# ChenYutongTHU/humannerf

Hardware: AMD Instinct MI355X
Metric: rendered rays/sec (128 samples/ray) at 512x512 (higher is better)
Workload: dtype f32-equivalent: split-f16 hi+lo operands, 3 f16 MFMAs, fp32 accumulate; 1 GPU; BASELINE configs[1]: 512x512 freeview frame, 262144 rays x 128 samples, eval, perturb=0, all 11 outputs of the reference Network.forward; seeded random weights of the default architecture; samples_per_ray=128, ray_chunk=32768, mlp_mode=f16x3, parallelism=frames sharded over 1 GPU(s), no collective

## Files before the change

### humannerf_amd/csrc/hnrf_mlp_f16.hip

```cpp
#include "hnrf_common.h"
#include "hnrf_sincos.h"
#include "hnrf_lds_dma.h"

namespace hnrf {

typedef float f32x16 __attribute__((ext_vector_type(16)));
typedef float f32x2 __attribute__((ext_vector_type(2)));
typedef _Float16 h16x8 __attribute__((ext_vector_type(8)));
typedef _Float16 h16x2 __attribute__((ext_vector_type(2)));

constexpr int RING = 3;
constexpr float LO_SCALE = 2048.0f;
constexpr float LO_INV = 1.0f / 2048.0f;

enum { PE16_NONE = 0, PE16_CANONICAL = 1, PE16_NONRIGID = 2 };

enum { SV_NONE = 0,
       SV_ACT = 1,
       SV_DZ = 2,
       SV_PE = 3,
       SV_ACT_H = 4,
       SV_DZ_H = 5 };
__host__ __device__ constexpr bool sv_fwd(int s) { return s == SV_ACT || s == SV_ACT_H; }
__host__ __device__ constexpr bool sv_bwd(int s) { return s == SV_DZ || s == SV_DZ_H; }
// ... 92 lines not shown
    }
    *reinterpret_cast<h16x2*>(dst) = h16x2{outv[0], outv[1]};
}

constexpr int64_t KB = 1024;
constexpr int CNL16_NB_L0 = 8, CNL16_NB_MID = 32, CNL16_NB_L5 = 40;
constexpr int64_t CNL16_L0 = 0;
constexpr int64_t CNL16_L1 = CNL16_L0 + 8 * CNL16_NB_L0 * KB;
constexpr int64_t CNL16_L5 = CNL16_L1 + 4 * 8 * CNL16_NB_MID * KB;
constexpr int64_t CNL16_L6 = CNL16_L5 + 8 * CNL16_NB_L5 * KB;
constexpr int64_t CNL16_OUT = CNL16_L6 + 2 * 8 * CNL16_NB_MID * KB;
constexpr int64_t CNL16_BIAS = CNL16_OUT + CNL16_NB_MID * KB;
constexpr int CNL16_BIAS_LDS = 8 * 1024;
constexpr int64_t CNL16_BYTES = CNL16_BIAS + 9 * 1024;
constexpr int CNL16_SLAB = 40 * 1024;
constexpr int NR16_NB_L0 = 8, NR16_NB_MID = 16, NR16_NB_L4 = 24;
constexpr int64_t NR16_L0 = 0;
constexpr int64_t NR16_L1 = NR16_L0 + 4 * NR16_NB_L0 * KB;
constexpr int64_t NR16_L4 = NR16_L1 + 3 * 4 * NR16_NB_MID * KB;
constexpr int64_t NR16_L5 = NR16_L4 + 4 * NR16_NB_L4 * KB;
constexpr int64_t NR16_OUT = NR16_L5 + 4 * NR16_NB_MID * KB;
constexpr int64_t NR16_BIAS = NR16_OUT + NR16_NB_MID * KB;
constexpr int NR16_BIAS_LDS = 3 * 1024;
constexpr int64_t NR16_BYTES = NR16_BIAS + 4 * 1024;
constexpr int NR16_SLAB = 32 * 1024;
constexpr int64_t CNL16_STATUS = CNL16_BIAS + 8 * 1024 + 512;
constexpr int64_t NR16_STATUS = NR16_BIAS + 3 * 1024 + 512;
constexpr int PE_STASH = 32 * 1024;

typedef __attribute__((address_space(3))) char lds_char;
typedef __attribute__((address_space(3))) h16x8 lds_h16x8;
typedef float f32x4 __attribute__((ext_vector_type(4)));
typedef __attribute__((address_space(3))) f32x4 lds_f32x4;

__device__ __forceinline__ h16x8 lds_ld8(unsigned addr) { return *reinterpret_cast<const lds_h16x8*>((size_t)addr); }
__device__ __forceinline__ f32x4 lds_ld4f(unsigned addr) { return *reinterpret_cast<const lds_f32x4*>((size_t)addr); }
__device__ __forceinline__ void lds_st8(unsigned addr, h16x8 v) { *reinterpret_cast<lds_h16x8*>((size_t)addr) = v; }

__device__ __forceinline__ void slab_issue(const char* gsrc, unsigned lds_addr, int nblocks, int wave, int nw = 4) {
    const unsigned voff = lane_now() * 16;
    for (int b = wave; b < nblocks; b += nw) dma_piece(gsrc + b * 1024, voff, lds_addr + b * 1024);
}

__device__ __forceinline__ void tile_sync(int keep) {
    wait_dma_keep(keep);
    __builtin_amdgcn_s_barrier();
    asm volatile("" ::: "memory");
}

template <bool ULO>
__device__ __forceinline__ void split8(const float (&v)[8], h16x8& hi, h16x8& lo) {
#pragma unroll
    for (int i = 0; i < 4; ++i) {
        const f32x2 p = {v[2 * i], v[2 * i + 1]};
        const h16x2 hh = __builtin_convertvector(p, h16x2);
        const f32x2 rem = ULO ? f32x2{p[0] - (float)hh[0], p[1] - (float)hh[1]}
                              : f32x2{fmaf((float)hh[0], -LO_SCALE, p[0] * LO_SCALE), fmaf((float)hh[1], -LO_SCALE, p[1] * LO_SCALE)};
// ... 152 lines not shown
        epi_core<ACT_MASK_SEL, ULO>(pacc1, pacc2, I, sc->mask[(T) >> 1] >> (16 * ((T) & 1)), 0, oh[2 * (T) + ((I) >> 2)],      \
                                    ol[2 * (T) + ((I) >> 2)], x0, x1);                                                         \
        save_pair_b(*sc, T, I, x0, x1);                                                                                        \
    } else if constexpr (SAVE == SV_DZ_H) {                                                                                    \
        float x0, x1;                                                                                                          \
        const h16x2 hh = epi_core<ACT_MASK_AND, ULO>(pacc1, pacc2, I, sc->mask[(T) >> 1], 8 * ((T) & 1) + (I),                 \
                                                     oh[2 * (T) + ((I) >> 2)], ol[2 * (T) + ((I) >> 2)], x0, x1);              \
        store_pair_h(rowh, cxh, svu, T, I, hh);                                                                                \
    } else if constexpr (SAVE == SV_PE) {                                                                                      \
        sc->fout[16 * (T) + 2 * (I)] = fmaf(pacc2[2 * (I)], LO_INV, pacc1[2 * (I)]);                                           \
        sc->fout[16 * (T) + 2 * (I) + 1] = fmaf(pacc2[2 * (I) + 1], LO_INV, pacc1[2 * (I) + 1]);                               \
    } else                                                                                                                     \
        epi_pair<RELU>(pacc1, I, oh[2 * (T) + ((I) >> 2)], ol[2 * (T) + ((I) >> 2)], p.sat, p.guard);

template <int NT, int TPS, int NKA, int NKB, bool RELU, int SAVE = 0, bool PEND_IN = false, bool DEFER = false,
          int NW = 4, int NB, int NO>
__device__ __forceinline__ void layer16(Pipe& p, int nb1, int nb2, h16x8 (&bh)[NB], h16x8 (&bl)[NB],
                                        h16x8 (&oh)[NO], h16x8 (&ol)[NO], float (&last)[16], SaveCtx* sc = nullptr,
                                        f32x16* pend = nullptr) {
    static_assert(!(PEND_IN || DEFER) || SAVE == SV_NONE, "deferred epilogues exist in the inference form only");
    static_assert(!PEND_IN || NKB >= 2, "a pending tile fills the last two hidden fragments");
    static_assert(NB >= (NKB > 0 ? NKB : 1) && NO >= 2 * NT && NT % TPS == 0, "bad layer shape");
    constexpr int NK = NKA + NKB;
    constexpr int NBLK = 2 * NK;
    constexpr int NS = NT / TPS;
    constexpr int PFK = NK < 4 ? NK : 4;
    static_assert((NBLK * TPS) % NW == 0, "every wave must issue the same number of DMA pieces per slab");
    constexpr bool ULO = !sv_lifted(SAVE);
    constexpr int ACT = RELU ? ACT_RELU : ACT_NONE;
    static_assert(ULO || NT > 1, "the head layers exist in the forward kernels only");
    f32x16 pacc1 = {0.f, 0.f, 0.f, 0.f, 0.f, 0.f, 0.f, 0.f, 0.f, 0.f, 0.f, 0.f, 0.f, 0.f, 0.f, 0.f};
    f32x16 pacc2 = pacc1;
    f32x16 nbias = pacc1;
    uint32_t bw[(NT + 1) / 2];
    _Float16* const rowh = (SAVE == SV_ACT_H || SAVE == SV_DZ_H) ? sc->rowh : nullptr;
    const int cxh = (SAVE == SV_ACT_H || SAVE == SV_DZ_H) ? sc->cx : 0;
    unsigned svu = 0u;
#pragma unroll
    for (int i = 0; i < (NT + 1) / 2; ++i) bw[i] = 0u;
#pragma unroll
    for (int s = 0; s < NS; ++s) {
        const int nissue = (s + 2 < NS) ? NBLK * TPS : (s + 2 == NS ? nb1 : nb2);
        const unsigned slot2 = p.ph == 0 ? 2 : p.ph - 1;
        const int dcnt = nissue / NW;
        const char* dsrc = p.gi + p.wave * dcnt * 1024;
        const unsigned ddst = p.lds_base + p.ring_off + slot2 * p.slab_bytes + p.wave * dcnt * 1024;
        p.gi += nissue * 1024;
#pragma unroll
        for (int tt = 0; tt < TPS; ++tt) {
            const int t = s * TPS + tt;
            const unsigned lane = lane_now();
            unsigned cur = p.lds_base + p.ring_off + p.ph * p.slab_bytes + tt * (NBLK * 1024) + lane * 16;
            unsigned pe = p.lds_base + p.pe_off + p.wave * (PE_STASH / 4) + lane * 16;
            asm volatile("" : "+v"(cur), "+v"(pe));
            f32x16 acc1 = {0.f, 0.f, 0.f, 0.f, 0.f, 0.f, 0.f, 0.f, 0.f, 0.f, 0.f, 0.f, 0.f, 0.f, 0.f, 0.f};
            f32x16 acc2 = acc1;
            if (NT > 1 && sv_has_bias(SAVE)) {
                if (t == 0) {
                    const unsigned bp = p.lds_base + p.bias_off + tt * 128 + (lane >> 5) * 16;
// ... 41 lines not shown
                if (ULO) acc1 = __builtin_amdgcn_mfma_f32_32x32x16_f16(wh, xl, acc1, 0, 0, 0);
                else acc2 = __builtin_amdgcn_mfma_f32_32x32x16_f16(wh, xl, acc2, 0, 0, 0);
                if (ULO) acc1 = __builtin_amdgcn_mfma_f32_32x32x16_f16(wl, xh, acc1, 0, 0, 0);
                else acc2 = __builtin_amdgcn_mfma_f32_32x32x16_f16(wl, xh, acc2, 0, 0, 0);
                if (NT > 1 && sv_has_bias(SAVE) && ks == NK - 1 && t + 1 < NT) {
                    const unsigned bn = p.lds_base + p.bias_off + (tt + 1) * 128 + (lane >> 5) * 16;
                    const f32x4 b0 = lds_ld4f(bn), b1 = lds_ld4f(bn + 32), b2 = lds_ld4f(bn + 64), b3 = lds_ld4f(bn + 96);
                    nbias = f32x16{b0.x, b0.y, b0.z, b0.w, b1.x, b1.y, b1.z, b1.w,
                                   b2.x, b2.y, b2.z, b2.w, b3.x, b3.y, b3.z, b3.w};
                }
                {
                    constexpr int MAXP = (TPS * NK - 1) < 10 ? (TPS * NK - 1) : 10;
                    const int i = tt * NK + ks;
                    if (i >= 0 && i < MAXP) {
                        if (s + 2 < NS) {
                            if (i < NBLK * TPS / NW) dma_run_piece(dsrc, lane * 16, ddst, i);
                        } else if (i < dcnt) {
                            dma_run_piece(dsrc, lane * 16, ddst, i);
                        }
                    }
                }
                if (PEND_IN && t == 0) {
#pragma unroll
                    for (int i = 0; i < 8; ++i)
                        if ((i * (NK - 1)) / 8 == ks) {
                            epi_pair<true>(*pend, i, bh[NKB - 2 + (i >> 2)], bl[NKB - 2 + (i >> 2)], p.sat, p.guard);
                            asm volatile("" : "+v"(bh[NKB - 2 + (i >> 2)]), "+v"(bl[NKB - 2 + (i >> 2)]));
                        }
                }
                if (t > 0) {
#pragma unroll
// ... 8 lines not shown
                __builtin_amdgcn_sched_group_barrier(0x002, 6, 0);
                __builtin_amdgcn_sched_group_barrier(0x008, 1, 0);
                __builtin_amdgcn_sched_group_barrier(0x100, 2, 0);
                __builtin_amdgcn_sched_group_barrier(0x002, 5, 0);
                __builtin_amdgcn_sched_group_barrier(0x008, 1, 0);
                __builtin_amdgcn_sched_group_barrier(0x002, 8, 0);
                __builtin_amdgcn_sched_barrier(0);
            }
#ifdef HNRF_STAMP
            { const unsigned long long t1 = __builtin_readcyclecounter(); p.sum_k += t1 - p.t_last; p.t_last = t1; }
#endif
            pacc1 = acc1;
            pacc2 = acc2;
        }
        const int n_st = (sv_fwd(SAVE) || sv_bwd(SAVE)) ? 4 * (s == 0 ? TPS - 1 : TPS) : 0;
        tile_sync(nissue / NW + n_st);
        p.ph = p.ph == RING - 1 ? 0 : p.ph + 1;
        p.bias_off += TPS * 128;
    }
    if (NT == 1) {
#pragma unroll
        for (int r = 0; r < 16; ++r) last[r] = pacc1[r];
    } else if (DEFER) {
        *pend = pacc1;
    } else {
#pragma unroll
        for (int i = 0; i < 8; ++i) {
            HNRF_TILE_EPILOGUE_PAIR(NT - 1, i)
        }
        if constexpr (sv_fwd(SAVE)) {
#pragma unroll
            for (int i = 0; i < (NT + 1) / 2; ++i) sc->bits[i] = bw[i];
        }
    }
}

#undef HNRF_TILE_EPILOGUE_PAIR

template <int NT, int TPS, int NKA, int NKB, bool RELU, int NB, int NO>
__device__ __forceinline__ void layer16x2(Pipe& p, unsigned stash_per_wave, int nb1, int nb2,
                                          const h16x8 (&bh)[2][NB], const h16x8 (&bl)[2][NB], h16x8 (&oh)[2][NO],
                                          h16x8 (&ol)[2][NO], float (&last)[2][16]) {
    static_assert(NB >= (NKB > 0 ? NKB : 1) && NO >= 2 * NT && NT % TPS == 0, "bad layer shape");
    constexpr int NK = NKA + NKB;
    constexpr int NBLK = 2 * NK;
    constexpr int NS = NT / TPS;
    constexpr int PFK = NK < 4 ? NK : 4;
    static_assert((NBLK * TPS) % 4 == 0, "every wave must issue the same number of DMA pieces per slab");
    const f32x16 zero = {0.f, 0.f, 0.f, 0.f, 0.f, 0.f, 0.f, 0.f, 0.f, 0.f, 0.f, 0.f, 0.f, 0.f, 0.f, 0.f};
    f32x16 pacc[2] = {zero, zero};
#pragma unroll
    for (int s = 0; s < NS; ++s) {
        const int nissue = (s + 2 < NS) ? NBLK * TPS : (s + 2 == NS ? nb1 : nb2);
        const unsigned slot2 = p.ph == 0 ? 2 : p.ph - 1;
        const int dcnt = nissue / 4;
        const char* dsrc = p.gi + p.wave * dcnt * 1024;
        const unsigned ddst = p.lds_base + p.ring_off + slot2 * p.slab_bytes + p.wave * dcnt * 1024;
        p.gi += nissue * 1024;
#pragma unroll
        for (int tt = 0; tt < TPS; ++tt) {
            const int t = s * TPS + tt;
            const unsigned lane = lane_now();
            unsigned cur = p.lds_base + p.ring_off + p.ph * p.slab_bytes + tt * (NBLK * 1024) + lane * 16;
            unsigned pe = p.lds_base + p.pe_off + p.wave * stash_per_wave + lane * 16;
            asm volatile("" : "+v"(cur), "+v"(pe));
            f32x16 acc[2] = {zero, zero};
            if (NT > 1) {
                const unsigned bp = p.lds_base + p.bias_off + tt * 128 + (lane >> 5) * 16;
                const f32x4 b0 = lds_ld4f(bp), b1 = lds_ld4f(bp + 32), b2 = lds_ld4f(bp + 64), b3 = lds_ld4f(bp + 96);
                acc[0] = f32x16{b0.x, b0.y, b0.z, b0.w, b1.x, b1.y, b1.z, b1.w,
                                 b2.x, b2.y, b2.z, b2.w, b3.x, b3.y, b3.z, b3.w};
                acc[1] = acc[0];
            }
            h16x8 qwh[PFK], qwl[PFK], qxh[2][PFK], qxl[2][PFK];
#pragma unroll
            for (int i = 0; i < PFK; ++i) {
                qwh[i] = lds_ld8(cur + (2 * i) * 1024);
                qwl[i] = lds_ld8(cur + (2 * i + 1) * 1024);
                if (i < NKA) {
#pragma unroll
                    for (int g = 0; g < 2; ++g) {
                        qxh[g][i] = lds_ld8(pe + g * (stash_per_wave / 2) + (2 * i) * 1024);
                        qxl[g][i] = lds_ld8(pe + g * (stash_per_wave / 2) + (2 * i + 1) * 1024);
                    }
                }
            }
            __builtin_amdgcn_sched_barrier(0);
#pragma unroll
            for (int ks = 0; ks < NK; ++ks) {
                const int q = ks % PFK;
                const h16x8 wh = qwh[q], wl = qwl[q];
                h16x8 xh[2], xl[2];
#pragma unroll
                for (int g = 0; g < 2; ++g) {
                    if (ks < NKA) {
                        xh[g] = qxh[g][q];
                        xl[g] = qxl[g][q];
                    } else {
                        const int ib = ks - NKA < NB ? ks - NKA : 0;
                        xh[g] = bh[g][ib];
                        xl[g] = bl[g][ib];
                    }
                }
                if (ks + PFK < NK) {
                    qwl[q] = lds_ld8(cur + (2 * (ks + PFK) + 1) * 1024);
                    if (ks + PFK < NKA) {
#pragma unroll
                        for (int g = 1; g >= 0; --g) qxl[g][q] = lds_ld8(pe + g * (stash_per_wave / 2) + (2 * (ks + PFK) + 1) * 1024);
                    }
                    qwh[q] = lds_ld8(cur + (2 * (ks + PFK)) * 1024);
                    if (ks + PFK < NKA) {
#pragma unroll
                        for (int g = 1; g >= 0; --g) qxh[g][q] = lds_ld8(pe + g * (stash_per_wave / 2) + (2 * (ks + PFK)) * 1024);
                    }
                }
#pragma unroll
                for (int g = 0; g < 2; ++g) {
                    acc[g] = __builtin_amdgcn_mfma_f32_32x32x16_f16(wh, xh[g], acc[g], 0, 0, 0);
                    acc[g] = __builtin_amdgcn_mfma_f32_32x32x16_f16(wh, xl[g], acc[g], 0, 0, 0);
                    acc[g] = __builtin_amdgcn_mfma_f32_32x32x16_f16(wl, xh[g], acc[g], 0, 0, 0);
                }
                {
                    constexpr int MAXP = (TPS * NK - 1) < 10 ? (TPS * NK - 1) : 10;
                    const int i = tt * NK + ks;
                    if (i >= 0 && i < MAXP) {
                        if (s + 2 < NS) {
                            if (i < NBLK * TPS / 4) dma_run_piece(dsrc, lane * 16, ddst, i);
                        } else if (i < dcnt) {
                            dma_run_piece(dsrc, lane * 16, ddst, i);
                        }
                    }
                }
                if (t > 0) {
#pragma unroll
                    for (int j = 0; j < 16; ++j)
                        if ((j * NK) / 16 == ks) {
                            const int g = j >> 3, i = j & 7;
                            epi_pair<RELU>(pacc[g], i, oh[g][2 * (t - 1) + (i >> 2)], ol[g][2 * (t - 1) + (i >> 2)], p.sat, p.guard);
                            asm volatile("" : "+v"(oh[g][2 * (t - 1) + (i >> 2)]), "+v"(ol[g][2 * (t - 1) + (i >> 2)]));
                        }
                }
                __builtin_amdgcn_sched_group_barrier(0x008, 1, 0);
                __builtin_amdgcn_sched_group_barrier(0x002, 6, 0);
                __builtin_amdgcn_sched_group_barrier(0x008, 1, 0);
                __builtin_amdgcn_sched_group_barrier(0x100, 2, 0);
                __builtin_amdgcn_sched_group_barrier(0x002, 5, 0);
                __builtin_amdgcn_sched_group_barrier(0x008, 1, 0);
                __builtin_amdgcn_sched_group_barrier(0x100, 2, 0);
                __builtin_amdgcn_sched_group_barrier(0x002, 5, 0);
                __builtin_amdgcn_sched_group_barrier(0x008, 1, 0);
                __builtin_amdgcn_sched_group_barrier(0x002, 6, 0);
                __builtin_amdgcn_sched_group_barrier(0x008, 1, 0);
                __builtin_amdgcn_sched_group_barrier(0x100, 2, 0);
                __builtin_amdgcn_sched_group_barrier(0x002, 5, 0);
                __builtin_amdgcn_sched_group_barrier(0x008, 1, 0);
                __builtin_amdgcn_sched_group_barrier(0x002, 8, 0);
                __builtin_amdgcn_sched_barrier(0);
            }
#pragma unroll
            for (int g = 0; g < 2; ++g) pacc[g] = acc[g];
        }
        tile_sync(nissue / 4);
        p.ph = p.ph == RING - 1 ? 0 : p.ph + 1;
        p.bias_off += TPS * 128;
    }
#pragma unroll
    for (int g = 0; g < 2; ++g) {
        if (NT == 1) {
#pragma unroll
            for (int r = 0; r < 16; ++r) last[g][r] = pacc[g][r];
        } else {
#pragma unroll
            for (int i = 0; i < 8; ++i)
                epi_pair<RELU>(pacc[g], i, oh[g][2 * (NT - 1) + (i >> 2)], ol[g][2 * (NT - 1) + (i >> 2)], p.sat, p.guard);
        }
    }
}

__device__ __forceinline__ Pipe pipe_start(const char* packed, int64_t bias_img_off, int bias_bytes, int slab_bytes,
                                           int nb0, int nb1, char* smem, int stash_bytes = PE_STASH, int nw = 4) {
    Pipe p;
    p.wave = __builtin_amdgcn_readfirstlane(threadIdx.x >> 6);
    p.lds_base = __builtin_amdgcn_readfirstlane((unsigned)(size_t)(lds_char*)smem);
    p.pe_off = bias_bytes;
    p.ring_off = bias_bytes + stash_bytes;
    p.slab_bytes = slab_bytes;
    p.ph = 0;
    p.bias_off = 0;
    p.sat = 0ull;
    p.guard = false;
#ifdef HNRF_STAMP
    p.t_last = __builtin_readcyclecounter();
// ... 95 lines not shown
    if (h == 0 && slot < P)
        raw[sample] = make_float4(fmaf(last[0], hs, ob[0]), fmaf(last[1], hs, ob[1]), fmaf(last[2], hs, ob[2]), fmaf(last[3], hs, ob[3]));
    if constexpr (SAVE == SV_NONE && GUARD) raise_f16_range(packed, CNL16_STATUS, p.sat);
#ifdef HNRF_STAMP
    if (threadIdx.x == 0 && blockIdx.x < 4096) {
        const unsigned long long te = __builtin_readcyclecounter();
        unsigned long long* dbg = (unsigned long long*)(const_cast<char*>(packed) + CNL16_BYTES);
        dbg[blockIdx.x * 4 + 0] = p.sum_k; dbg[blockIdx.x * 4 + 1] = p.sum_b + (te - p.t_last);
    }
#endif
}

constexpr int NR16W8_SLAB = 24 * 1024;
constexpr int NR16W8_STASH = 64 * 1024;

template <int SAVE, int NW = 4>
__global__ __launch_bounds__(64 * NW) void nonrigid_f16x3_kernel(const float* __restrict__ x_skel,
                                                             const float* __restrict__ hann_w,
                                                             const char* __restrict__ packed, int64_t P,
                                                             float* __restrict__ xyz, float* __restrict__ offsets,
                                                             const int* __restrict__ idx,
                                                             const int* __restrict__ count,
                                                             float* __restrict__ pe_out, float* __restrict__ acts,
                                                             uint32_t* __restrict__ relu_bits) {
    extern __shared__ __attribute__((aligned(16))) char smem[];
    if (idx != nullptr) {
        P = *count;
        if ((int64_t)blockIdx.x * (32 * NW) >= P) return;
    }
    static_assert(NW == 4 || NW == 8, "waves per workgroup");
    constexpr bool W8 = NW == 8;
    Pipe p = W8 ? pipe_start(packed, NR16_BIAS, NR16_BIAS_LDS, NR16W8_SLAB, 2 * NR16_NB_L0, 2 * NR16_NB_L0, smem, NR16W8_STASH, 8)
                : pipe_start(packed, NR16_BIAS, NR16_BIAS_LDS, NR16_SLAB, 4 * NR16_NB_L0, 2 * NR16_NB_MID, smem);
    const int lane = threadIdx.x & 63, h = lane >> 5;
    const int64_t slot = ((int64_t)blockIdx.x * NW + p.wave) * 32 + (lane & 31);
    const int64_t sclamp = slot < P ? slot : P - 1;
    const int64_t sidx = idx ? (int64_t)idx[sclamp] : sclamp;
    const int64_t sample = slot < P ? sidx : P;

    const float x[3] = {x_skel[sidx * 3 + 0], x_skel[sidx * 3 + 1], x_skel[sidx * 3 + 2]};
    float pev[32];
    pe_sincos_shared<6>(x, h, pev);
#pragma unroll
    for (int a = 0; a < 18; ++a) pev[a] *= hann_w[a / 3];
#pragma unroll
    for (int a = 18; a < 32; ++a) pev[a] = 0.f;
#pragma unroll
    for (int ks = 0; ks < 4; ++ks) {
        const float v[8] = {pev[8 * ks], pev[8 * ks + 1], pev[8 * ks + 2], pev[8 * ks + 3],
                            pev[8 * ks + 4], pev[8 * ks + 5], pev[8 * ks + 6], pev[8 * ks + 7]};
        stash_pe<true>(p, ks, v);
    }
    SaveCtx sc;
    if constexpr (SAVE) {
        sc.row = acts + sidx * 128 + 4 * h;
        sc.rowh = reinterpret_cast<_Float16*>(acts) + (slot >> 5) * (128 * 32) + h * 128;
        sc.cx = (lane & 31) ^ (4 * h);
        sc.bits = relu_bits + sidx * 4 + 2 * h;
        if constexpr (SAVE == SV_ACT_H) {
            _Float16* ph = reinterpret_cast<_Float16*>(pe_out) + sidx * 64;
#pragma unroll
            for (int a = 0; a < 18; ++a) ph[pe_col16(PE16_NONRIGID, a, h)] = (_Float16)pev[a];
#pragma unroll
            for (int a = 18; a < 32; ++a) ph[36 + 2 * (a - 18) + h] = (_Float16)0.f;
        } else {
#pragma unroll
            for (int a = 0; a < 18; ++a) pe_out[sidx * 36 + pe_col16(PE16_NONRIGID, a, h)] = pev[a];
        }
    }
    const int64_t act_stride = P * 128, bit_stride = P * 4;
    const int64_t acth_stride = (int64_t)gridDim.x * (32 * NW) * 128;
    tile_sync(0);

    h16x8 hA_h[8], hA_l[8], hB_h[8], hB_l[8];
    float last[16];
    h16x8 dh[2], dl[2];
    if constexpr (W8) {
        constexpr int MID = NR16_NB_MID, L4B = NR16_NB_L4;
#define HNRF_NEXT_LAYER if constexpr (SAVE) { sc.row += act_stride; sc.rowh += acth_stride; sc.bits += bit_stride; }
        layer16<4, 2, 4, 0, true, SAVE, false, false, 8>(p, MID, MID, hB_h, hB_l, hA_h, hA_l, last, &sc);
        HNRF_NEXT_LAYER
        layer16<4, 1, 0, 8, true, SAVE, false, false, 8>(p, MID, MID, hA_h, hA_l, hB_h, hB_l, last, &sc);
        HNRF_NEXT_LAYER
        layer16<4, 1, 0, 8, true, SAVE, false, false, 8>(p, MID, MID, hB_h, hB_l, hA_h, hA_l, last, &sc);
        HNRF_NEXT_LAYER
        layer16<4, 1, 0, 8, true, SAVE, false, false, 8>(p, L4B, L4B, hA_h, hA_l, hB_h, hB_l, last, &sc);
        HNRF_NEXT_LAYER
        layer16<4, 1, 4, 8, true, SAVE, false, false, 8>(p, MID, MID, hB_h, hB_l, hA_h, hA_l, last, &sc);
        HNRF_NEXT_LAYER
        layer16<4, 1, 0, 8, true, SAVE, false, false, 8>(p, MID, 0, hA_h, hA_l, hB_h, hB_l, last, &sc);
#undef HNRF_NEXT_LAYER
        layer16<1, 1, 0, 8, false, 0, false, false, 8>(p, 0, 0, hB_h, hB_l, dh, dl, last);
    } else {
    layer16<4, 4, 4, 0, true, SAVE>(p, 0 , 2 * NR16_NB_MID, hB_h, hB_l, hA_h, hA_l, last, &sc);
    if constexpr (SAVE) { sc.row += act_stride; sc.rowh += acth_stride; sc.bits += bit_stride; }
    layer16<4, 2, 0, 8, true, SAVE>(p, 2 * NR16_NB_MID, 2 * NR16_NB_MID, hA_h, hA_l, hB_h, hB_l, last, &sc);
    if constexpr (SAVE) { sc.row += act_stride; sc.rowh += acth_stride; sc.bits += bit_stride; }
    layer16<4, 2, 0, 8, true, SAVE>(p, 2 * NR16_NB_MID, 2 * NR16_NB_MID, hB_h, hB_l, hA_h, hA_l, last, &sc);
    if constexpr (SAVE) { sc.row += act_stride; sc.rowh += acth_stride; sc.bits += bit_stride; }
    layer16<4, 2, 0, 8, true, SAVE>(p, NR16_NB_L4, NR16_NB_L4, hA_h, hA_l, hB_h, hB_l, last, &sc);
    if constexpr (SAVE) { sc.row += act_stride; sc.rowh += acth_stride; sc.bits += bit_stride; }
    layer16<4, 1, 4, 8, true, SAVE>(p, 2 * NR16_NB_MID, 2 * NR16_NB_MID, hB_h, hB_l, hA_h, hA_l, last, &sc);
    if constexpr (SAVE) { sc.row += act_stride; sc.rowh += acth_stride; sc.bits += bit_stride; }
    layer16<4, 2, 0, 8, true, SAVE>(p, NR16_NB_MID, 0, hA_h, hA_l, hB_h, hB_l, last, &sc);
    layer16<1, 1, 0, 8, false, 0>(p, 0, 0, hB_h, hB_l, dh, dl, last);
    }
    const float* ob = reinterpret_cast<const float*>(packed + NR16_BIAS + NR16_BIAS_LDS);
    const float hs = ob[8];
    if (h == 0 && slot < P) {
        const float o0 = fmaf(last[0], hs, ob[0]), o1 = fmaf(last[1], hs, ob[1]), o2 = fmaf(last[2], hs, ob[2]);
        xyz[sample * 3 + 0] = x[0] + o0;
        xyz[sample * 3 + 1] = x[1] + o1;
        xyz[sample * 3 + 2] = x[2] + o2;
        if (offsets) {
            offsets[sample * 3 + 0] = o0;
            offsets[sample * 3 + 1] = o1;
            offsets[sample * 3 + 2] = o2;
        }
    }
}

constexpr int NR16X2_SLAB = 24 * 1024;
constexpr int NR16X2_STASH = 64 * 1024;

template <bool GUARD>
__global__ __launch_bounds__(256) void nonrigid_f16x3_x2_kernel(const float* __restrict__ x_skel,
                                                                const float* __restrict__ hann_w,
                                                                const char* __restrict__ packed, int64_t P,
                                                                float* __restrict__ xyz, float* __restrict__ offsets,
                                                                const int* __restrict__ idx,
                                                                const int* __restrict__ count) {
    extern __shared__ __attribute__((aligned(16))) char smem[];
    if (idx != nullptr) {
        P = *count;
        if ((int64_t)blockIdx.x * 256 >= P) return;
    }
    Pipe p = pipe_start(packed, NR16_BIAS, NR16_BIAS_LDS, NR16X2_SLAB, 2 * NR16_NB_L0, 2 * NR16_NB_L0, smem,
                        NR16X2_STASH);
    p.guard = GUARD;
    constexpr unsigned SPW = NR16X2_STASH / 4;
    const int lane = threadIdx.x & 63, h = lane >> 5;
    int64_t sidx[2];
    bool live[2];
    float x[2][3];
#pragma unroll
    for (int g = 0; g < 2; ++g) {
        const int64_t slot = ((int64_t)blockIdx.x * 4 + p.wave) * 64 + g * 32 + (lane & 31);
        const int64_t sclamp = slot < P ? slot : P - 1;
        sidx[g] = idx ? (int64_t)idx[sclamp] : sclamp;
        live[g] = slot < P;
#pragma unroll
        for (int a = 0; a < 3; ++a) x[g][a] = x_skel[sidx[g] * 3 + a];
    }
#pragma unroll
    for (int g = 0; g < 2; ++g) {
        float pev[32];
        pe_sincos_shared<6>(x[g], h, pev);
#pragma unroll
        for (int a = 0; a < 18; ++a) pev[a] *= hann_w[a / 3];
#pragma unroll
        for (int a = 18; a < 32; ++a) pev[a] = 0.f;
        const unsigned pe = p.lds_base + p.pe_off + p.wave * SPW + g * (SPW / 2) + lane_now() * 16;
#pragma unroll
        for (int ks = 0; ks < 4; ++ks) {
            const float v[8] = {pev[8 * ks], pev[8 * ks + 1], pev[8 * ks + 2], pev[8 * ks + 3],
                                pev[8 * ks + 4], pev[8 * ks + 5], pev[8 * ks + 6], pev[8 * ks + 7]};
            h16x8 hi, lo;
            split8<true>(v, hi, lo);
            lds_st8(pe + (2 * ks) * 1024, hi);
            lds_st8(pe + (2 * ks + 1) * 1024, lo);
        }
    }
    tile_sync(0);

    h16x8 hA_h[2][8], hA_l[2][8], hB_h[2][8], hB_l[2][8];
    float last[2][16];
    constexpr int MID = NR16_NB_MID, L4B = NR16_NB_L4;
    layer16x2<4, 2, 4, 0, true>(p, SPW, MID, MID, hB_h, hB_l, hA_h, hA_l, last);
    layer16x2<4, 1, 0, 8, true>(p, SPW, MID, MID, hA_h, hA_l, hB_h, hB_l, last);
    layer16x2<4, 1, 0, 8, true>(p, SPW, MID, MID, hB_h, hB_l, hA_h, hA_l, last);
    layer16x2<4, 1, 0, 8, true>(p, SPW, L4B, L4B, hA_h, hA_l, hB_h, hB_l, last);
    layer16x2<4, 1, 4, 8, true>(p, SPW, MID, MID, hB_h, hB_l, hA_h, hA_l, last);
    layer16x2<4, 1, 0, 8, true>(p, SPW, MID, 0, hA_h, hA_l, hB_h, hB_l, last);
    h16x8 dh[2][2], dl[2][2];
    layer16x2<1, 1, 0, 8, false>(p, SPW, 0, 0, hB_h, hB_l, dh, dl, last);
    const float* ob = reinterpret_cast<const float*>(packed + NR16_BIAS + NR16_BIAS_LDS);
    const float hs = ob[8];
#pragma unroll
    for (int g = 0; g < 2; ++g) {
        if (h == 0 && live[g]) {
            const float o0 = fmaf(last[g][0], hs, ob[0]), o1 = fmaf(last[g][1], hs, ob[1]), o2 = fmaf(last[g][2], hs, ob[2]);
            xyz[sidx[g] * 3 + 0] = x[g][0] + o0;
            xyz[sidx[g] * 3 + 1] = x[g][1] + o1;
            xyz[sidx[g] * 3 + 2] = x[g][2] + o2;
            if (offsets) {
                offsets[sidx[g] * 3 + 0] = o0;
                offsets[sidx[g] * 3 + 1] = o1;
                offsets[sidx[g] * 3 + 2] = o2;
            }
        }
    }
    if constexpr (GUARD) raise_f16_range(packed, NR16_STATUS, p.sat);
}

struct PackBwd16 {
    const float* W;
    int n_out, n_in;
    int NT, NK;
    int row_kind;
    int col0;
    int head;
    int64_t off;
    const float* amax;
};
// ... 340 lines not shown
    d[5] = PackLayer16{w[5], b[5], 256, 319, 8, 4, 16, PE16_CANONICAL, 0, 63, 0, CNL16_L5, CNL16_BIAS + 5 * 1024, 0};
    for (int l = 6; l <= 7; ++l)
        d[l] = PackLayer16{w[l], b[l], 256, 256, 8, 0, 16, PE16_NONE, 0, 0, 0,
                           CNL16_L6 + (l - 6) * 8 * CNL16_NB_MID * KB, CNL16_BIAS + l * 1024, 0};
    d[8] = PackLayer16{w[8], b[8], 4, 256, 1, 0, 16, PE16_NONE, 0, 0, 0, CNL16_OUT, CNL16_BIAS + 8 * 1024, 1};
    return launch_pack16(d, 9, nullptr, out, st);
}

int nonrigid16_pack(const float* const* w, const float* const* b, const float* cond, void* packed, hipStream_t st) {
    char* out = (char*)packed;
    if (hipMemsetAsync(out + NR16_BIAS, 0, 4 * 1024, st) != hipSuccess) {
        set_error("hnrf_nonrigid_pack: memset failed");
        return HNRF_E_LAUNCH;
    }
    PackLayer16 d[7];
    d[0] = PackLayer16{w[0], b[0], 128, 105, 4, 4, 0, PE16_NONRIGID, 69, 0, 69, NR16_L0, NR16_BIAS, 0};
    for (int l = 1; l <= 3; ++l)
        d[l] = PackLayer16{w[l], b[l], 128, 128, 4, 0, 8, PE16_NONE, 0, 0, 0,
                           NR16_L1 + (l - 1) * 4 * NR16_NB_MID * KB, NR16_BIAS + l * 512, 0};
    d[4] = PackLayer16{w[4], b[4], 128, 164, 4, 4, 8, PE16_NONRIGID, 128, 0, 0, NR16_L4, NR16_BIAS + 4 * 512, 0};
    d[5] = PackLayer16{w[5], b[5], 128, 128, 4, 0, 8, PE16_NONE, 0, 0, 0, NR16_L5, NR16_BIAS + 5 * 512, 0};
    d[6] = PackLayer16{w[6], b[6], 3, 128, 1, 0, 8, PE16_NONE, 0, 0, 0, NR16_OUT, NR16_BIAS + 6 * 512, 1};
    return launch_pack16(d, 7, cond, out, st);
}

int canonical16_fwd(const float* xyz, const void* packed, int64_t P, float* raw, const int* idx, const int* count,
                    bool guard, hipStream_t st) {
    constexpr int lds = CNL16_BIAS_LDS + PE_STASH + RING * CNL16_SLAB;
    const dim3 grid((unsigned)((P + 127) / 128));
    const char* what = "hnrf_canonical_fwd (f16x3)";
    if (guard)
        return launch_lds<canonical_f16x3_kernel<SV_NONE, true>>(what, grid, dim3(256), lds, st, xyz, (const char*)packed, P,
                                                                 (float4*)raw, idx, count, nullptr, nullptr, nullptr);
    return launch_lds<canonical_f16x3_kernel<SV_NONE, false>>(what, grid, dim3(256), lds, st, xyz, (const char*)packed, P,
                                                              (float4*)raw, idx, count, nullptr, nullptr, nullptr);
// ... 1 lines not shown

int canonical16_fwd_train(const float* xyz, const void* packed, int64_t P, float* raw, float* pe_out, float* acts,
                          uint32_t* relu_bits, int half, hipStream_t st) {
    constexpr int lds = CNL16_BIAS_LDS + PE_STASH + RING * CNL16_SLAB;
    const dim3 grid((unsigned)((P + 127) / 128));
    const char* what = "hnrf_canonical_fwd_train (f16x3)";
    if (half)
        return launch_lds<canonical_f16x3_kernel<SV_ACT_H>>(what, grid, dim3(256), lds, st, xyz, (const char*)packed, P,
                                                            (float4*)raw, nullptr, nullptr, pe_out, acts, relu_bits);
    return launch_lds<canonical_f16x3_kernel<SV_ACT>>(what, grid, dim3(256), lds, st, xyz, (const char*)packed, P, (float4*)raw,
                                                      nullptr, nullptr, pe_out, acts, relu_bits);
}

int nonrigid16_fwd(const float* x_skel, const float* hann_w, const void* packed, int64_t P, float* xyz,
                   float* offsets, const int* idx, const int* count, bool guard, hipStream_t st) {
    constexpr int lds2 = NR16_BIAS_LDS + NR16X2_STASH + RING * NR16X2_SLAB;
    const dim3 grid((unsigned)((P + 255) / 256));
    const char* what = "hnrf_nonrigid_fwd (f16x3)";
    if (guard)
        return launch_lds<nonrigid_f16x3_x2_kernel<true>>(what, grid, dim3(256), lds2, st, x_skel, hann_w, (const char*)packed, P,
                                                          xyz, offsets, idx, count);
    return launch_lds<nonrigid_f16x3_x2_kernel<false>>(what, grid, dim3(256), lds2, st, x_skel, hann_w, (const char*)packed, P,
                                                       xyz, offsets, idx, count);
}

int nonrigid16_fwd_train(const float* x_skel, const float* hann_w, const void* packed, int64_t P, float* xyz,
                         float* offsets, float* pe_out, float* acts, uint32_t* relu_bits, int half, hipStream_t st) {
    constexpr int lds = NR16_BIAS_LDS + PE_STASH + RING * NR16_SLAB;
    const dim3 grid((unsigned)((P + 127) / 128));
    const char* what = "hnrf_nonrigid_fwd_train (f16x3)";
    if (half && P % 256 == 0) {
        constexpr int lds8 = NR16_BIAS_LDS + NR16W8_STASH + RING * NR16W8_SLAB;
        return launch_lds<nonrigid_f16x3_kernel<SV_ACT_H, 8>>(what, dim3((unsigned)(P / 256)), dim3(512), lds8, st, x_skel, hann_w,
                                                              (const char*)packed, P, xyz, offsets, nullptr, nullptr, pe_out,
                                                              acts, relu_bits);
    }
    if (half)
        return launch_lds<nonrigid_f16x3_kernel<SV_ACT_H>>(what, grid, dim3(256), lds, st, x_skel, hann_w, (const char*)packed, P,
// ... 93 lines not shown
```

Before: 5.027 million rays/s.

## Trim nonrigid PE K-steps to three and run inference on 8-wave kernel

Shrinks the nonrigid MLP's positional-encoding input from four to three 16-wide K fragments, since only 18 PE values are real. This cuts weight bytes and MFMAs in layers 0 and 4, and a padded DMA mode handles slab piece counts that no longer divide evenly across waves. The separate two-group x2 inference kernel is removed. Inference now uses the 8-wave nonrigid kernel with a guard template flag. The risk is that uneven DMA piece counts and the different wave organisation could change pipelining and occupancy.

```diff
diff --git a/humannerf_amd/csrc/hnrf_mlp_f16.hip b/humannerf_amd/csrc/hnrf_mlp_f16.hip
--- a/humannerf_amd/csrc/hnrf_mlp_f16.hip
+++ b/humannerf_amd/csrc/hnrf_mlp_f16.hip
@@ -130,7 +130,8 @@
 constexpr int CNL16_BIAS_LDS = 8 * 1024;
 constexpr int64_t CNL16_BYTES = CNL16_BIAS + 9 * 1024;
 constexpr int CNL16_SLAB = 40 * 1024;
-constexpr int NR16_NB_L0 = 8, NR16_NB_MID = 16, NR16_NB_L4 = 24;
+constexpr int NR16_NKA = 3;
+constexpr int NR16_NB_L0 = 6, NR16_NB_MID = 16, NR16_NB_L4 = 22;
 constexpr int64_t NR16_L0 = 0;
 constexpr int64_t NR16_L1 = NR16_L0 + 4 * NR16_NB_L0 * KB;
 constexpr int64_t NR16_L4 = NR16_L1 + 3 * 4 * NR16_NB_MID * KB;
@@ -157,6 +158,8 @@
     const unsigned voff = lane_now() * 16;
     for (int b = wave; b < nblocks; b += nw) dma_piece(gsrc + b * 1024, voff, lds_addr + b * 1024);
 }
+
+__host__ __device__ constexpr int slab_pieces(int nblocks, int nw) { return (nblocks + nw - 1) / nw; }
 
 __device__ __forceinline__ void tile_sync(int keep) {
     wait_dma_keep(keep);
@@ -339,7 +342,7 @@
         epi_pair<RELU>(pacc1, I, oh[2 * (T) + ((I) >> 2)], ol[2 * (T) + ((I) >> 2)], p.sat, p.guard);
 
 template <int NT, int TPS, int NKA, int NKB, bool RELU, int SAVE = 0, bool PEND_IN = false, bool DEFER = false,
-          int NW = 4, int NB, int NO>
+          int NW = 4, bool PADDED = false, int NB, int NO>
 __device__ __forceinline__ void layer16(Pipe& p, int nb1, int nb2, h16x8 (&bh)[NB], h16x8 (&bl)[NB],
                                         h16x8 (&oh)[NO], h16x8 (&ol)[NO], float (&last)[16], SaveCtx* sc = nullptr,
                                         f32x16* pend = nullptr) {
@@ -350,7 +353,9 @@
     constexpr int NBLK = 2 * NK;
     constexpr int NS = NT / TPS;
     constexpr int PFK = NK < 4 ? NK : 4;
-    static_assert((NBLK * TPS) % NW == 0, "every wave must issue the same number of DMA pieces per slab");
+    static_assert(PADDED || (NBLK * TPS) % NW == 0, "every wave must issue the same number of DMA pieces per slab");
+    constexpr int NPCS = slab_pieces(NBLK * TPS, NW);
+    static_assert(NS <= 2 || NPCS <= ((TPS * NK - 1) < 10 ? (TPS * NK - 1) : 10), "more DMA pieces per wave than k-steps that issue them");
     constexpr bool ULO = !sv_lifted(SAVE);
     constexpr int ACT = RELU ? ACT_RELU : ACT_NONE;
     static_assert(ULO || NT > 1, "the head layers exist in the forward kernels only");
@@ -367,7 +372,7 @@
     for (int s = 0; s < NS; ++s) {
         const int nissue = (s + 2 < NS) ? NBLK * TPS : (s + 2 == NS ? nb1 : nb2);
         const unsigned slot2 = p.ph == 0 ? 2 : p.ph - 1;
-        const int dcnt = nissue / NW;
+        const int dcnt = PADDED ? slab_pieces(nissue, NW) : nissue / NW;
         const char* dsrc = p.gi + p.wave * dcnt * 1024;
         const unsigned ddst = p.lds_base + p.ring_off + slot2 * p.slab_bytes + p.wave * dcnt * 1024;
         p.gi += nissue * 1024;
@@ -439,7 +444,7 @@
                     const int i = tt * NK + ks;
                     if (i >= 0 && i < MAXP) {
                         if (s + 2 < NS) {
-                            if (i < NBLK * TPS / NW) dma_run_piece(dsrc, lane * 16, ddst, i);
+                            if (i < NPCS) dma_run_piece(dsrc, lane * 16, ddst, i);
                         } else if (i < dcnt) {
                             dma_run_piece(dsrc, lane * 16, ddst, i);
                         }
@@ -478,7 +483,7 @@
             pacc2 = acc2;
         }
         const int n_st = (sv_fwd(SAVE) || sv_bwd(SAVE)) ? 4 * (s == 0 ? TPS - 1 : TPS) : 0;
-        tile_sync(nissue / NW + n_st);
+        tile_sync(dcnt + n_st);
         p.ph = p.ph == RING - 1 ? 0 : p.ph + 1;
         p.bias_off += TPS * 128;
     }
@@ -500,146 +505,6 @@
 }
 
 #undef HNRF_TILE_EPILOGUE_PAIR
-
-template <int NT, int TPS, int NKA, int NKB, bool RELU, int NB, int NO>
-__device__ __forceinline__ void layer16x2(Pipe& p, unsigned stash_per_wave, int nb1, int nb2,
-                                          const h16x8 (&bh)[2][NB], const h16x8 (&bl)[2][NB], h16x8 (&oh)[2][NO],
-                                          h16x8 (&ol)[2][NO], float (&last)[2][16]) {
-    static_assert(NB >= (NKB > 0 ? NKB : 1) && NO >= 2 * NT && NT % TPS == 0, "bad layer shape");
-    constexpr int NK = NKA + NKB;
-    constexpr int NBLK = 2 * NK;
-    constexpr int NS = NT / TPS;
-    constexpr int PFK = NK < 4 ? NK : 4;
-    static_assert((NBLK * TPS) % 4 == 0, "every wave must issue the same number of DMA pieces per slab");
-    const f32x16 zero = {0.f, 0.f, 0.f, 0.f, 0.f, 0.f, 0.f, 0.f, 0.f, 0.f, 0.f, 0.f, 0.f, 0.f, 0.f, 0.f};
-    f32x16 pacc[2] = {zero, zero};
-#pragma unroll
-    for (int s = 0; s < NS; ++s) {
-        const int nissue = (s + 2 < NS) ? NBLK * TPS : (s + 2 == NS ? nb1 : nb2);
-        const unsigned slot2 = p.ph == 0 ? 2 : p.ph - 1;
-        const int dcnt = nissue / 4;
-        const char* dsrc = p.gi + p.wave * dcnt * 1024;
-        const unsigned ddst = p.lds_base + p.ring_off + slot2 * p.slab_bytes + p.wave * dcnt * 1024;
-        p.gi += nissue * 1024;
-#pragma unroll
-        for (int tt = 0; tt < TPS; ++tt) {
-            const int t = s * TPS + tt;
-            const unsigned lane = lane_now();
-            unsigned cur = p.lds_base + p.ring_off + p.ph * p.slab_bytes + tt * (NBLK * 1024) + lane * 16;
-            unsigned pe = p.lds_base + p.pe_off + p.wave * stash_per_wave + lane * 16;
-            asm volatile("" : "+v"(cur), "+v"(pe));
-            f32x16 acc[2] = {zero, zero};
-            if (NT > 1) {
-                const unsigned bp = p.lds_base + p.bias_off + tt * 128 + (lane >> 5) * 16;
-                const f32x4 b0 = lds_ld4f(bp), b1 = lds_ld4f(bp + 32), b2 = lds_ld4f(bp + 64), b3 = lds_ld4f(bp + 96);
-                acc[0] = f32x16{b0.x, b0.y, b0.z, b0.w, b1.x, b1.y, b1.z, b1.w,
-                                 b2.x, b2.y, b2.z, b2.w, b3.x, b3.y, b3.z, b3.w};
-                acc[1] = acc[0];
-            }
-            h16x8 qwh[PFK], qwl[PFK], qxh[2][PFK], qxl[2][PFK];
-#pragma unroll
-            for (int i = 0; i < PFK; ++i) {
-                qwh[i] = lds_ld8(cur + (2 * i) * 1024);
-                qwl[i] = lds_ld8(cur + (2 * i + 1) * 1024);
-                if (i < NKA) {
-#pragma unroll
-                    for (int g = 0; g < 2; ++g) {
-                        qxh[g][i] = lds_ld8(pe + g * (stash_per_wave / 2) + (2 * i) * 1024);
-                        qxl[g][i] = lds_ld8(pe + g * (stash_per_wave / 2) + (2 * i + 1) * 1024);
-                    }
-                }
-            }
-            __builtin_amdgcn_sched_barrier(0);
-#pragma unroll
-            for (int ks = 0; ks < NK; ++ks) {
-                const int q = ks % PFK;
-                const h16x8 wh = qwh[q], wl = qwl[q];
-                h16x8 xh[2], xl[2];
-#pragma unroll
-                for (int g = 0; g < 2; ++g) {
-                    if (ks < NKA) {
-                        xh[g] = qxh[g][q];
-                        xl[g] = qxl[g][q];
-                    } else {
-                        const int ib = ks - NKA < NB ? ks - NKA : 0;
-                        xh[g] = bh[g][ib];
-                        xl[g] = bl[g][ib];
-                    }
-                }
-                if (ks + PFK < NK) {
-                    qwl[q] = lds_ld8(cur + (2 * (ks + PFK) + 1) * 1024);
-                    if (ks + PFK < NKA) {
-#pragma unroll
-                        for (int g = 1; g >= 0; --g) qxl[g][q] = lds_ld8(pe + g * (stash_per_wave / 2) + (2 * (ks + PFK) + 1) * 1024);
-                    }
-                    qwh[q] = lds_ld8(cur + (2 * (ks + PFK)) * 1024);
-                    if (ks + PFK < NKA) {
-#pragma unroll
-                        for (int g = 1; g >= 0; --g) qxh[g][q] = lds_ld8(pe + g * (stash_per_wave / 2) + (2 * (ks + PFK)) * 1024);
-                    }
-                }
-#pragma unroll
-                for (int g = 0; g < 2; ++g) {
-                    acc[g] = __builtin_amdgcn_mfma_f32_32x32x16_f16(wh, xh[g], acc[g], 0, 0, 0);
-                    acc[g] = __builtin_amdgcn_mfma_f32_32x32x16_f16(wh, xl[g], acc[g], 0, 0, 0);
-                    acc[g] = __builtin_amdgcn_mfma_f32_32x32x16_f16(wl, xh[g], acc[g], 0, 0, 0);
-                }
-                {
-                    constexpr int MAXP = (TPS * NK - 1) < 10 ? (TPS * NK - 1) : 10;
-                    const int i = tt * NK + ks;
-                    if (i >= 0 && i < MAXP) {
-                        if (s + 2 < NS) {
-                            if (i < NBLK * TPS / 4) dma_run_piece(dsrc, lane * 16, ddst, i);
-                        } else if (i < dcnt) {
-                            dma_run_piece(dsrc, lane * 16, ddst, i);
-                        }
-                    }
-                }
-                if (t > 0) {
-#pragma unroll
-                    for (int j = 0; j < 16; ++j)
-                        if ((j * NK) / 16 == ks) {
-                            const int g = j >> 3, i = j & 7;
-                            epi_pair<RELU>(pacc[g], i, oh[g][2 * (t - 1) + (i >> 2)], ol[g][2 * (t - 1) + (i >> 2)], p.sat, p.guard);
-                            asm volatile("" : "+v"(oh[g][2 * (t - 1) + (i >> 2)]), "+v"(ol[g][2 * (t - 1) + (i >> 2)]));
-                        }
-                }
-                __builtin_amdgcn_sched_group_barrier(0x008, 1, 0);
-                __builtin_amdgcn_sched_group_barrier(0x002, 6, 0);
-                __builtin_amdgcn_sched_group_barrier(0x008, 1, 0);
-                __builtin_amdgcn_sched_group_barrier(0x100, 2, 0);
-                __builtin_amdgcn_sched_group_barrier(0x002, 5, 0);
-                __builtin_amdgcn_sched_group_barrier(0x008, 1, 0);
-                __builtin_amdgcn_sched_group_barrier(0x100, 2, 0);
-                __builtin_amdgcn_sched_group_barrier(0x002, 5, 0);
-                __builtin_amdgcn_sched_group_barrier(0x008, 1, 0);
-                __builtin_amdgcn_sched_group_barrier(0x002, 6, 0);
-                __builtin_amdgcn_sched_group_barrier(0x008, 1, 0);
-                __builtin_amdgcn_sched_group_barrier(0x100, 2, 0);
-                __builtin_amdgcn_sched_group_barrier(0x002, 5, 0);
-                __builtin_amdgcn_sched_group_barrier(0x008, 1, 0);
-                __builtin_amdgcn_sched_group_barrier(0x002, 8, 0);
-                __builtin_amdgcn_sched_barrier(0);
-            }
-#pragma unroll
-            for (int g = 0; g < 2; ++g) pacc[g] = acc[g];
-        }
-        tile_sync(nissue / 4);
-        p.ph = p.ph == RING - 1 ? 0 : p.ph + 1;
-        p.bias_off += TPS * 128;
-    }
-#pragma unroll
-    for (int g = 0; g < 2; ++g) {
-        if (NT == 1) {
-#pragma unroll
-            for (int r = 0; r < 16; ++r) last[g][r] = pacc[g][r];
-        } else {
-#pragma unroll
-            for (int i = 0; i < 8; ++i)
-                epi_pair<RELU>(pacc[g], i, oh[g][2 * (NT - 1) + (i >> 2)], ol[g][2 * (NT - 1) + (i >> 2)], p.sat, p.guard);
-        }
-    }
-}
 
 __device__ __forceinline__ Pipe pipe_start(const char* packed, int64_t bias_img_off, int bias_bytes, int slab_bytes,
                                            int nb0, int nb1, char* smem, int stash_bytes = PE_STASH, int nw = 4) {
@@ -765,7 +630,7 @@
 constexpr int NR16W8_SLAB = 24 * 1024;
 constexpr int NR16W8_STASH = 64 * 1024;
 
-template <int SAVE, int NW = 4>
+template <int SAVE, int NW = 4, bool GUARD = false>
 __global__ __launch_bounds__(64 * NW) void nonrigid_f16x3_kernel(const float* __restrict__ x_skel,
                                                              const float* __restrict__ hann_w,
                                                              const char* __restrict__ packed, int64_t P,
@@ -783,6 +648,8 @@
     constexpr bool W8 = NW == 8;
     Pipe p = W8 ? pipe_start(packed, NR16_BIAS, NR16_BIAS_LDS, NR16W8_SLAB, 2 * NR16_NB_L0, 2 * NR16_NB_L0, smem, NR16W8_STASH, 8)
                 : pipe_start(packed, NR16_BIAS, NR16_BIAS_LDS, NR16_SLAB, 4 * NR16_NB_L0, 2 * NR16_NB_MID, smem);
+    static_assert(!GUARD || SAVE == SV_NONE, "the range guard belongs to the inference form");
+    p.guard = GUARD;
     const int lane = threadIdx.x & 63, h = lane >> 5;
     const int64_t slot = ((int64_t)blockIdx.x * NW + p.wave) * 32 + (lane & 31);
     const int64_t sclamp = slot < P ? slot : P - 1;
@@ -790,14 +657,14 @@
     const int64_t sample = slot < P ? sidx : P;
 
     const float x[3] = {x_skel[sidx * 3 + 0], x_skel[sidx * 3 + 1], x_skel[sidx * 3 + 2]};
-    float pev[32];
+    float pev[8 * NR16_NKA];
     pe_sincos_shared<6>(x, h, pev);
 #pragma unroll
     for (int a = 0; a < 18; ++a) pev[a] *= hann_w[a / 3];
 #pragma unroll
-    for (int a = 18; a < 32; ++a) pev[a] = 0.f;
-#pragma unroll
-    for (int ks = 0; ks < 4; ++ks) {
+    for (int a = 18; a < 8 * NR16_NKA; ++a) pev[a] = 0.f;
+#pragma unroll
+    for (int ks = 0; ks < NR16_NKA; ++ks) {
         const float v[8] = {pev[8 * ks], pev[8 * ks + 1], pev[8 * ks + 2], pev[8 * ks + 3],
                             pev[8 * ks + 4], pev[8 * ks + 5], pev[8 * ks + 6], pev[8 * ks + 7]};
         stash_pe<true>(p, ks, v);
@@ -813,7 +680,7 @@
 #pragma unroll
             for (int a = 0; a < 18; ++a) ph[pe_col16(PE16_NONRIGID, a, h)] = (_Float16)pev[a];
 #pragma unroll
-            for (int a = 18; a < 32; ++a) ph[36 + 2 * (a - 18) + h] = (_Float16)0.f;
+            for (int c = 36; c < 64; c += 2) ph[c + h] = (_Float16)0.f;
         } else {
 #pragma unroll
             for (int a = 0; a < 18; ++a) pe_out[sidx * 36 + pe_col16(PE16_NONRIGID, a, h)] = pev[a];
@@ -829,29 +696,29 @@
     if constexpr (W8) {
         constexpr int MID = NR16_NB_MID, L4B = NR16_NB_L4;
 #define HNRF_NEXT_LAYER if constexpr (SAVE) { sc.row += act_stride; sc.rowh += acth_stride; sc.bits += bit_stride; }
-        layer16<4, 2, 4, 0, true, SAVE, false, false, 8>(p, MID, MID, hB_h, hB_l, hA_h, hA_l, last, &sc);
+        layer16<4, 2, NR16_NKA, 0, true, SAVE, false, false, 8, true>(p, MID, MID, hB_h, hB_l, hA_h, hA_l, last, &sc);
         HNRF_NEXT_LAYER
         layer16<4, 1, 0, 8, true, SAVE, false, false, 8>(p, MID, MID, hA_h, hA_l, hB_h, hB_l, last, &sc);
         HNRF_NEXT_LAYER
         layer16<4, 1, 0, 8, true, SAVE, false, false, 8>(p, MID, MID, hB_h, hB_l, hA_h, hA_l, last, &sc);
         HNRF_NEXT_LAYER
-        layer16<4, 1, 0, 8, true, SAVE, false, false, 8>(p, L4B, L4B, hA_h, hA_l, hB_h, hB_l, last, &sc);
+        layer16<4, 1, 0, 8, true, SAVE, false, false, 8, true>(p, L4B, L4B, hA_h, hA_l, hB_h, hB_l, last, &sc);
         HNRF_NEXT_LAYER
-        layer16<4, 1, 4, 8, true, SAVE, false, false, 8>(p, MID, MID, hB_h, hB_l, hA_h, hA_l, last, &sc);
+        layer16<4, 1, NR16_NKA, 8, true, SAVE, false, false, 8, true>(p, MID, MID, hB_h, hB_l, hA_h, hA_l, last, &sc);
         HNRF_NEXT_LAYER
         layer16<4, 1, 0, 8, true, SAVE, false, false, 8>(p, MID, 0, hA_h, hA_l, hB_h, hB_l, last, &sc);
 #undef HNRF_NEXT_LAYER
         layer16<1, 1, 0, 8, false, 0, false, false, 8>(p, 0, 0, hB_h, hB_l, dh, dl, last);
     } else {
-    layer16<4, 4, 4, 0, true, SAVE>(p, 0 , 2 * NR16_NB_MID, hB_h, hB_l, hA_h, hA_l, last, &sc);
+    layer16<4, 4, NR16_NKA, 0, true, SAVE>(p, 0 , 2 * NR16_NB_MID, hB_h, hB_l, hA_h, hA_l, last, &sc);
     if constexpr (SAVE) { sc.row += act_stride; sc.rowh += acth_stride; sc.bits += bit_stride; }
     layer16<4, 2, 0, 8, true, SAVE>(p, 2 * NR16_NB_MID, 2 * NR16_NB_MID, hA_h, hA_l, hB_h, hB_l, last, &sc);
     if constexpr (SAVE) { sc.row += act_stride; sc.rowh += acth_stride; sc.bits += bit_stride; }
     layer16<4, 2, 0, 8, true, SAVE>(p, 2 * NR16_NB_MID, 2 * NR16_NB_MID, hB_h, hB_l, hA_h, hA_l, last, &sc);
     if constexpr (SAVE) { sc.row += act_stride; sc.rowh += acth_stride; sc.bits += bit_stride; }
-    layer16<4, 2, 0, 8, true, SAVE>(p, NR16_NB_L4, NR16_NB_L4, hA_h, hA_l, hB_h, hB_l, last, &sc);
+    layer16<4, 2, 0, 8, true, SAVE, false, false, 4, true>(p, NR16_NB_L4, NR16_NB_L4, hA_h, hA_l, hB_h, hB_l, last, &sc);
     if constexpr (SAVE) { sc.row += act_stride; sc.rowh += acth_stride; sc.bits += bit_stride; }
-    layer16<4, 1, 4, 8, true, SAVE>(p, 2 * NR16_NB_MID, 2 * NR16_NB_MID, hB_h, hB_l, hA_h, hA_l, last, &sc);
+    layer16<4, 1, NR16_NKA, 8, true, SAVE, false, false, 4, true>(p, 2 * NR16_NB_MID, 2 * NR16_NB_MID, hB_h, hB_l, hA_h, hA_l, last, &sc);
     if constexpr (SAVE) { sc.row += act_stride; sc.rowh += acth_stride; sc.bits += bit_stride; }
     layer16<4, 2, 0, 8, true, SAVE>(p, NR16_NB_MID, 0, hA_h, hA_l, hB_h, hB_l, last, &sc);
     layer16<1, 1, 0, 8, false, 0>(p, 0, 0, hB_h, hB_l, dh, dl, last);
@@ -867,88 +734,6 @@
             offsets[sample * 3 + 0] = o0;
             offsets[sample * 3 + 1] = o1;
             offsets[sample * 3 + 2] = o2;
-        }
-    }
-}
-
-constexpr int NR16X2_SLAB = 24 * 1024;
-constexpr int NR16X2_STASH = 64 * 1024;
-
-template <bool GUARD>
-__global__ __launch_bounds__(256) void nonrigid_f16x3_x2_kernel(const float* __restrict__ x_skel,
-                                                                const float* __restrict__ hann_w,
-                                                                const char* __restrict__ packed, int64_t P,
-                                                                float* __restrict__ xyz, float* __restrict__ offsets,
-                                                                const int* __restrict__ idx,
-                                                                const int* __restrict__ count) {
-    extern __shared__ __attribute__((aligned(16))) char smem[];
-    if (idx != nullptr) {
-        P = *count;
-        if ((int64_t)blockIdx.x * 256 >= P) return;
-    }
-    Pipe p = pipe_start(packed, NR16_BIAS, NR16_BIAS_LDS, NR16X2_SLAB, 2 * NR16_NB_L0, 2 * NR16_NB_L0, smem,
-                        NR16X2_STASH);
-    p.guard = GUARD;
-    constexpr unsigned SPW = NR16X2_STASH / 4;
-    const int lane = threadIdx.x & 63, h = lane >> 5;
-    int64_t sidx[2];
-    bool live[2];
-    float x[2][3];
-#pragma unroll
-    for (int g = 0; g < 2; ++g) {
-        const int64_t slot = ((int64_t)blockIdx.x * 4 + p.wave) * 64 + g * 32 + (lane & 31);
-        const int64_t sclamp = slot < P ? slot : P - 1;
-        sidx[g] = idx ? (int64_t)idx[sclamp] : sclamp;
-        live[g] = slot < P;
-#pragma unroll
-        for (int a = 0; a < 3; ++a) x[g][a] = x_skel[sidx[g] * 3 + a];
-    }
-#pragma unroll
-    for (int g = 0; g < 2; ++g) {
-        float pev[32];
-        pe_sincos_shared<6>(x[g], h, pev);
-#pragma unroll
-        for (int a = 0; a < 18; ++a) pev[a] *= hann_w[a / 3];
-#pragma unroll
-        for (int a = 18; a < 32; ++a) pev[a] = 0.f;
-        const unsigned pe = p.lds_base + p.pe_off + p.wave * SPW + g * (SPW / 2) + lane_now() * 16;
-#pragma unroll
-        for (int ks = 0; ks < 4; ++ks) {
-            const float v[8] = {pev[8 * ks], pev[8 * ks + 1], pev[8 * ks + 2], pev[8 * ks + 3],
-                                pev[8 * ks + 4], pev[8 * ks + 5], pev[8 * ks + 6], pev[8 * ks + 7]};
-            h16x8 hi, lo;
-            split8<true>(v, hi, lo);
-            lds_st8(pe + (2 * ks) * 1024, hi);
-            lds_st8(pe + (2 * ks + 1) * 1024, lo);
-        }
-    }
-    tile_sync(0);
-
-    h16x8 hA_h[2][8], hA_l[2][8], hB_h[2][8], hB_l[2][8];
-    float last[2][16];
-    constexpr int MID = NR16_NB_MID, L4B = NR16_NB_L4;
-    layer16x2<4, 2, 4, 0, true>(p, SPW, MID, MID, hB_h, hB_l, hA_h, hA_l, last);
-    layer16x2<4, 1, 0, 8, true>(p, SPW, MID, MID, hA_h, hA_l, hB_h, hB_l, last);
-    layer16x2<4, 1, 0, 8, true>(p, SPW, MID, MID, hB_h, hB_l, hA_h, hA_l, last);
-    layer16x2<4, 1, 0, 8, true>(p, SPW, L4B, L4B, hA_h, hA_l, hB_h, hB_l, last);
-    layer16x2<4, 1, 4, 8, true>(p, SPW, MID, MID, hB_h, hB_l, hA_h, hA_l, last);
-    layer16x2<4, 1, 0, 8, true>(p, SPW, MID, 0, hA_h, hA_l, hB_h, hB_l, last);
-    h16x8 dh[2][2], dl[2][2];
-    layer16x2<1, 1, 0, 8, false>(p, SPW, 0, 0, hB_h, hB_l, dh, dl, last);
-    const float* ob = reinterpret_cast<const float*>(packed + NR16_BIAS + NR16_BIAS_LDS);
-    const float hs = ob[8];
-#pragma unroll
-    for (int g = 0; g < 2; ++g) {
-        if (h == 0 && live[g]) {
-            const float o0 = fmaf(last[g][0], hs, ob[0]), o1 = fmaf(last[g][1], hs, ob[1]), o2 = fmaf(last[g][2], hs, ob[2]);
-            xyz[sidx[g] * 3 + 0] = x[g][0] + o0;
-            xyz[sidx[g] * 3 + 1] = x[g][1] + o1;
-            xyz[sidx[g] * 3 + 2] = x[g][2] + o2;
-            if (offsets) {
-                offsets[sidx[g] * 3 + 0] = o0;
-                offsets[sidx[g] * 3 + 1] = o1;
-                offsets[sidx[g] * 3 + 2] = o2;
-            }
         }
     }
     if constexpr (GUARD) raise_f16_range(packed, NR16_STATUS, p.sat);
@@ -1319,11 +1104,11 @@
         return HNRF_E_LAUNCH;
     }
     PackLayer16 d[7];
-    d[0] = PackLayer16{w[0], b[0], 128, 105, 4, 4, 0, PE16_NONRIGID, 69, 0, 69, NR16_L0, NR16_BIAS, 0};
+    d[0] = PackLayer16{w[0], b[0], 128, 105, 4, NR16_NKA, 0, PE16_NONRIGID, 69, 0, 69, NR16_L0, NR16_BIAS, 0};
     for (int l = 1; l <= 3; ++l)
         d[l] = PackLayer16{w[l], b[l], 128, 128, 4, 0, 8, PE16_NONE, 0, 0, 0,
                            NR16_L1 + (l - 1) * 4 * NR16_NB_MID * KB, NR16_BIAS + l * 512, 0};
-    d[4] = PackLayer16{w[4], b[4], 128, 164, 4, 4, 8, PE16_NONRIGID, 128, 0, 0, NR16_L4, NR16_BIAS + 4 * 512, 0};
+    d[4] = PackLayer16{w[4], b[4], 128, 164, 4, NR16_NKA, 8, PE16_NONRIGID, 128, 0, 0, NR16_L4, NR16_BIAS + 4 * 512, 0};
     d[5] = PackLayer16{w[5], b[5], 128, 128, 4, 0, 8, PE16_NONE, 0, 0, 0, NR16_L5, NR16_BIAS + 5 * 512, 0};
     d[6] = PackLayer16{w[6], b[6], 3, 128, 1, 0, 8, PE16_NONE, 0, 0, 0, NR16_OUT, NR16_BIAS + 6 * 512, 1};
     return launch_pack16(d, 7, cond, out, st);
@@ -1355,14 +1140,14 @@
 
 int nonrigid16_fwd(const float* x_skel, const float* hann_w, const void* packed, int64_t P, float* xyz,
                    float* offsets, const int* idx, const int* count, bool guard, hipStream_t st) {
-    constexpr int lds2 = NR16_BIAS_LDS + NR16X2_STASH + RING * NR16X2_SLAB;
+    constexpr int lds8 = NR16_BIAS_LDS + NR16W8_STASH + RING * NR16W8_SLAB;
     const dim3 grid((unsigned)((P + 255) / 256));
     const char* what = "hnrf_nonrigid_fwd (f16x3)";
     if (guard)
-        return launch_lds<nonrigid_f16x3_x2_kernel<true>>(what, grid, dim3(256), lds2, st, x_skel, hann_w, (const char*)packed, P,
-                                                          xyz, offsets, idx, count);
-    return launch_lds<nonrigid_f16x3_x2_kernel<false>>(what, grid, dim3(256), lds2, st, x_skel, hann_w, (const char*)packed, P,
-                                                       xyz, offsets, idx, count);
+        return launch_lds<nonrigid_f16x3_kernel<SV_NONE, 8, true>>(what, grid, dim3(512), lds8, st, x_skel, hann_w, (const char*)packed,
+                                                                   P, xyz, offsets, idx, count, nullptr, nullptr, nullptr);
+    return launch_lds<nonrigid_f16x3_kernel<SV_NONE, 8, false>>(what, grid, dim3(512), lds8, st, x_skel, hann_w, (const char*)packed,
+                                                                P, xyz, offsets, idx, count, nullptr, nullptr, nullptr);
 }
 
 int nonrigid16_fwd_train(const float* x_skel, const float* hann_w, const void* packed, int64_t P, float* xyz,
```

New measurement: 5.059 million rays/s, median of 6. Within noise of the previous version (+0.6%).
